# jiaxiZeng/Temporally-Consistent-Stereo-Matching

Measured on AMD Instinct MI355X. Metric: stereo-pairs/sec at 640x480 D=192, 32 GRU iters, higher is better.
Workload: dtype f32; 1 GPU; BASELINE configs[1]: 640x480 synthetic sequence len=10, D=192, 32 iters, one sequence per GPU; frames_per_rank=87, seqs_per_gpu=1, weights=key-seeded synthetic (tcs_mi355.weights)

## Files before the change

### include/tcs_mi355.h

```cpp
#ifndef TCS_MI355_H
#define TCS_MI355_H

#include <stddef.h>
#include <stdint.h>

#ifdef __cplusplus
extern "C" {
#endif

#define TCS_OK 0
#define TCS_EINVAL (-1)
#define TCS_ELAUNCH (-2)
#define TCS_EUNSUPPORTED (-3)

typedef void* tcs_stream_t;

int tcs_abi_version(void);
const char* tcs_error_string(int code);


size_t tcs_corr_level_bytes(int B, int H, int W, int level);
size_t tcs_corr_build_workspace_bytes(int B, int H, int W);

int tcs_corr_build(const float* fmap1, const float* fmap2, int B, int C, int H, int W,
                   float* pyr0, float* pyr1, float* pyr2, float* pyr3,
                   float* nat1, float* nat2, float* nat3,
                   float* cost_volume,
                   float* sparse_disp, float* sparse_cost, float* sparse_mask,
                   void* workspace, tcs_stream_t stream);
float* tcs_corr_ws_level0(void* workspace);

int tcs_corr_lookup(const float* pyr0, const float* pyr1, const float* pyr2, const float* pyr3,
                    const float* coords, int B, int H, int W, int radius, float* out,
                    unsigned long long* stamps, tcs_stream_t stream);
int tcs_corr_lookup_blocks(int B, int H, int W);

int tcs_corr_lookup_backward(const float* pyr0, const float* pyr1, const float* pyr2, const float* pyr3,
                             const float* coords, const float* grad_out, int B, int H, int W, int radius,
                             float* grad_vol, float* grad_coords, tcs_stream_t stream);

size_t tcs_corr_build_backward_scratch_bytes(int B, int C, int H, int W);
int tcs_corr_build_backward(const float* fmap1, const float* fmap2, const void* workspace, const float* grad_vol,
                            int B, int C, int H, int W, float* grad_fmap1, float* grad_fmap2, void* scratch,
                            tcs_stream_t stream);

size_t tcs_warp_workspace_bytes(int B, int C, int H, int W);

int tcs_warp_forward(const float* prev_disp, const float* prev_fmap, const float* T_rel, const float* K,
                     const float* K_inv, const float* baseline, int B, int C, int H, int W,
                     float* out_disp, float* out_fmap, float* out_mask,
                     const float* cur_fmap, float* out_cost,
// ... 301 lines not shown
```

### temporally-consistent-stereo-matching_amd/csrc/tcs_s16_ops.hip

```cpp
#include "tcs_s16.h"

__global__ __launch_bounds__(256) void k_avgpool3s2_s16(const _Float16* __restrict__ x, int G, int H, int W, int Ho, int Wo,
                                                         _Float16* __restrict__ out, int Go) {
    const int bg = blockIdx.y, b = bg / G, g = bg - b * G;
    const int p = blockIdx.x * 256 + threadIdx.x;
    if (p >= Ho * Wo) return;
    const int yo = p / Wo, xo = p - yo * Wo;
    const int Hp = H + 2, Wp = W + 2;
    const size_t plane = (size_t)Hp * Wp * 8;
    const _Float16* s = x + (((size_t)b * G + g) * 2) * plane;
    float acc[8] = {0.f, 0.f, 0.f, 0.f, 0.f, 0.f, 0.f, 0.f};
#pragma unroll
    for (int v = 0; v < 3; ++v) {
#pragma unroll
        for (int u = 0; u < 3; ++u) {
            float t[8];
            s16_load8(s + ((size_t)(2 * yo + v) * Wp + (2 * xo + u)) * 8, plane, t);
#pragma unroll
            for (int j = 0; j < 8; ++j) acc[j] += t[j];
        }
    }
#pragma unroll
    for (int j = 0; j < 8; ++j) acc[j] = acc[j] / 9.f;
    s16_store8(out + s16_unit(b, Go, g, 0, Ho + 2, Wo + 2, yo, xo), (size_t)(Ho + 2) * (Wo + 2) * 8, acc);
}

__global__ __launch_bounds__(256) void k_resize_bilinear_s16(const _Float16* __restrict__ x, int G, int H, int W, int Ho, int Wo,
                                                              _Float16* __restrict__ out, int Go) {
    const int bg = blockIdx.y, b = bg / G, g = bg - b * G;
    const int p = blockIdx.x * 256 + threadIdx.x;
    if (p >= Ho * Wo) return;
    const int yo = p / Wo, xo = p - yo * Wo;
    const float sy = Ho > 1 ? (float)(H - 1) / (float)(Ho - 1) : 0.f;
    const float sx = Wo > 1 ? (float)(W - 1) / (float)(Wo - 1) : 0.f;
    const float fy = sy * (float)yo, fx = sx * (float)xo;
    const int y0 = (int)fy, x0 = (int)fx;
    const int y1 = y0 + (y0 < H - 1), x1 = x0 + (x0 < W - 1);
    const float ly = fy - (float)y0, lx = fx - (float)x0;
    const int Hp = H + 2, Wp = W + 2;
    const size_t plane = (size_t)Hp * Wp * 8;
    const _Float16* s = x + (((size_t)b * G + g) * 2) * plane;
    float a00[8], a01[8], a10[8], a11[8], r[8];
    s16_load8(s + ((size_t)(y0 + 1) * Wp + x0 + 1) * 8, plane, a00);
    s16_load8(s + ((size_t)(y0 + 1) * Wp + x1 + 1) * 8, plane, a01);
    s16_load8(s + ((size_t)(y1 + 1) * Wp + x0 + 1) * 8, plane, a10);
    s16_load8(s + ((size_t)(y1 + 1) * Wp + x1 + 1) * 8, plane, a11);
#pragma unroll
    for (int j = 0; j < 8; ++j) r[j] = (1.f - ly) * ((1.f - lx) * a00[j] + lx * a01[j]) + ly * ((1.f - lx) * a10[j] + lx * a11[j]);
    s16_store8(out + s16_unit(b, Go, g, 0, Ho + 2, Wo + 2, yo, xo), (size_t)(Ho + 2) * (Wo + 2) * 8, r);
}

#define INS_T 256
#define INS_UPT 10

__device__ __forceinline__ void block_sum8(float* v, float* red ) {
#pragma unroll
    for (int j = 0; j < 8; ++j) v[j] = wave_sum(v[j]);
    __syncthreads();
    if ((threadIdx.x & 63) == 0) {
#pragma unroll
        for (int j = 0; j < 8; ++j) red[(threadIdx.x >> 6) * 8 + j] = v[j];
    }
    __syncthreads();
#pragma unroll
    for (int j = 0; j < 8; ++j) {
        float s = 0.f;
#pragma unroll
        for (int w = 0; w < INS_T / 64; ++w) s += red[w * 8 + j];
        v[j] = s;
    }
}

__global__ __launch_bounds__(INS_T) void k_in_stats_s16(const _Float16* __restrict__ x, int G, int H, int W, int slice_px,
                                                         float* __restrict__ partial ) {
    __shared__ float red[(INS_T / 64) * 8];
    const int bg = blockIdx.y, sl = blockIdx.x, nsl = gridDim.x;
    const int HW = H * W, Wp = W + 2;
    const size_t plane = (size_t)(H + 2) * Wp * 8;
    const _Float16* s = x + ((size_t)bg * 2) * plane;
    const int p_lo = sl * slice_px, p_hi = min(HW, p_lo + slice_px), n = p_hi - p_lo;
    float v[INS_UPT][8], sum[8] = {0.f, 0.f, 0.f, 0.f, 0.f, 0.f, 0.f, 0.f};
#pragma unroll
    for (int k = 0; k < INS_UPT; ++k) {
        const int p = p_lo + threadIdx.x + INS_T * k;
        const bool ok = p < p_hi;
        const int pc = ok ? p : p_lo;
        const int y = pc / W, xx = pc - y * W;
        s16_load8(s + ((size_t)(y + 1) * Wp + xx + 1) * 8, plane, v[k]);
#pragma unroll
        for (int j = 0; j < 8; ++j) { v[k][j] = ok ? v[k][j] : 0.f; sum[j] += v[k][j]; }
    }
    block_sum8(sum, red);
    float mean[8], m2[8] = {0.f, 0.f, 0.f, 0.f, 0.f, 0.f, 0.f, 0.f};
#pragma unroll
    for (int j = 0; j < 8; ++j) mean[j] = sum[j] / (float)n;
#pragma unroll
    for (int k = 0; k < INS_UPT; ++k) {
        const bool ok = p_lo + threadIdx.x + INS_T * k < p_hi;
#pragma unroll
        for (int j = 0; j < 8; ++j) { const float d = ok ? v[k][j] - mean[j] : 0.f; m2[j] = fmaf(d, d, m2[j]); }
    }
    block_sum8(m2, red);
    if (threadIdx.x < 8) {
        float* o = partial + ((size_t)bg * nsl + sl) * 16;
        o[threadIdx.x] = mean[threadIdx.x];
        o[8 + threadIdx.x] = m2[threadIdx.x];
    }
}

__device__ __forceinline__ float s16_act(float v, int act) {
    switch (act) {
        case TCS_ACT_RELU: return fmaxf(v, 0.f);
        case TCS_ACT_RELU_ADD_RELU: return fmaxf(v, 0.f);
        case TCS_ACT_LEAKY: return v > 0.f ? v : 0.01f * v;
        default: return v;
    }
}

__global__ __launch_bounds__(INS_T) void k_in_apply_s16(const _Float16* __restrict__ x, int G, int H, int W, int slice_px, int nsl,
                                                         const float* __restrict__ partial, float eps, int act,
                                                         const _Float16* __restrict__ addend, int Ga, _Float16* __restrict__ out, int Go) {
    const int bg = blockIdx.y, b = bg / G, g = bg - b * G;
    const int HW = H * W, Wp = W + 2;
    const size_t plane = (size_t)(H + 2) * Wp * 8;
    const int p = blockIdx.x * INS_T + threadIdx.x;
    const bool ok = p < HW;
    const int pc = ok ? p : HW - 1;
    const int y = pc / W, xx = pc - y * W;
    const size_t u = ((size_t)(y + 1) * Wp + xx + 1) * 8;
    float v[8], t[8];
    s16_load8(x + ((size_t)bg * 2) * plane + u, plane, v);
    if (addend) s16_load8(addend + (((size_t)b * Ga + g) * 2) * plane + u, plane, t);
    float n = 0.f, mean[8], m2[8];
#pragma unroll
    for (int j = 0; j < 8; ++j) { mean[j] = 0.f; m2[j] = 0.f; }
#pragma unroll 4
    for (int i = 0; i < nsl; ++i) {
        const float4* pi = reinterpret_cast<const float4*>(partial + ((size_t)bg * nsl + i) * 16);
        const float4 a0 = pi[0], a1 = pi[1], q0 = pi[2], q1 = pi[3];
        const float pm[8] = {a0.x, a0.y, a0.z, a0.w, a1.x, a1.y, a1.z, a1.w}, p2[8] = {q0.x, q0.y, q0.z, q0.w, q1.x, q1.y, q1.z, q1.w};
        const float ni = (float)(min(HW, (i + 1) * slice_px) - i * slice_px), tot = n + ni, f = ni / tot;
#pragma unroll
        for (int j = 0; j < 8; ++j) {
            const float d = pm[j] - mean[j];
            mean[j] += d * f;
            m2[j] += p2[j] + d * d * n * f;
        }
        n = tot;
    }
    if (!ok) return;
#pragma unroll
    for (int j = 0; j < 8; ++j) {
        const float rstd = 1.0f / sqrtf(m2[j] / (float)HW + eps);
        v[j] = s16_act((v[j] - mean[j]) * rstd, act) + (addend ? t[j] : 0.f);
        if (act == TCS_ACT_RELU_ADD_RELU) v[j] = fmaxf(v[j], 0.f);
    }
    s16_store8(out + (((size_t)b * Go + g) * 2) * plane + u, plane, v);
}

__global__ __launch_bounds__(INS_T) void k_in_apply_sums_s16(const _Float16* __restrict__ x, int Gt, int G, int H, int W, int C,
                                                              const long long* __restrict__ sums, float eps, int act,
                                                              const _Float16* __restrict__ addend, int Ga, _Float16* __restrict__ out, int Go) {
    const int b = blockIdx.y / G, g = blockIdx.y - b * G, bg = b * Gt + g;
    const int HW = H * W, Wp = W + 2;
    const size_t plane = (size_t)(H + 2) * Wp * 8;
    const int p = blockIdx.x * INS_T + threadIdx.x;
    if (p >= HW) return;
    const int y = p / W, xx = p - y * W;
    const size_t u = ((size_t)(y + 1) * Wp + xx + 1) * 8;
    float v[8], t[8];
    s16_load8(x + ((size_t)bg * 2) * plane + u, plane, v);
    if (addend) s16_load8(addend + (((size_t)b * Ga + g) * 2) * plane + u, plane, t);
    const long long* sp = sums + ((size_t)b * C + min(g * 8, C - 8)) * S16_IN_STRIDE;
    const double inv_n = 1.0 / (double)HW;
#pragma unroll
    for (int j = 0; j < 8; ++j) {
        const double mu = (double)sp[S16_IN_STRIDE * j] * (inv_n / 1048576.0), ex2 = (double)sp[S16_IN_STRIDE * j + 1] * (inv_n / 65536.0);
        const float mean = (float)mu, rstd = 1.0f / sqrtf(fmaxf((float)(ex2 - mu * mu), 0.f) + eps);
        const bool real = g * 8 + j < C;
        v[j] = real ? s16_act((v[j] - mean) * rstd, act) + (addend ? t[j] : 0.f) : 0.f;
        if (act == TCS_ACT_RELU_ADD_RELU) v[j] = fmaxf(v[j], 0.f);
    }
    s16_store8(out + (((size_t)b * Go + g) * 2) * plane + u, plane, v);
}

__global__ __launch_bounds__(256) void k_propagate_s16(const float* __restrict__ grad, const float* __restrict__ disp, int H, int W,
                                                        float* __restrict__ cand9, _Float16* __restrict__ out16, int Go) {
    const int b = blockIdx.y, HW = H * W;
    const int p = blockIdx.x * 256 + threadIdx.x;
    if (p >= HW) return;
// ... 114 lines not shown
}

__global__ __launch_bounds__(256) void k_s16_set_channel(const float* __restrict__ x, int H, int W, _Float16* __restrict__ out, int Go, int ch) {
    const int b = blockIdx.y, HW = H * W;
    const int p = blockIdx.x * 256 + threadIdx.x;
    if (p >= HW) return;
    const int y = p / W, xx = p - y * W;
    half2_t hi, lo;
    s16_split2(x[(size_t)b * HW + p], 0.f, hi, lo);
    _Float16* o = out + s16_unit(b, Go, ch >> 3, 0, H + 2, W + 2, y, xx) + (ch & 7);
    o[0] = hi[0];
    o[(size_t)(H + 2) * (W + 2) * 8] = lo[0];
}

extern "C" {

int tcs_avgpool3s2_s16(const void* x, int B, int groups, int H, int W, void* out, int out_groups, tcs_stream_t stream) {
    if (!x || !out || B <= 0 || groups <= 0 || out_groups < groups || H <= 0 || W <= 0) return TCS_EINVAL;
    if ((long long)B * groups > 65535) return TCS_EUNSUPPORTED;
    const int Ho = (H - 1) / 2 + 1, Wo = (W - 1) / 2 + 1;
    hipLaunchKernelGGL(k_avgpool3s2_s16, dim3(tcs_cdiv((long long)Ho * Wo, 256), B * groups), dim3(256), 0, tcs_stream(stream),
                       reinterpret_cast<const _Float16*>(x), groups, H, W, Ho, Wo, reinterpret_cast<_Float16*>(out), out_groups);
    return tcs_launch_status();
}

int tcs_resize_bilinear_s16(const void* x, int B, int groups, int H, int W, int Ho, int Wo, void* out, int out_groups, tcs_stream_t stream) {
    if (!x || !out || B <= 0 || groups <= 0 || out_groups < groups || H <= 0 || W <= 0 || Ho <= 0 || Wo <= 0) return TCS_EINVAL;
    if ((long long)B * groups > 65535) return TCS_EUNSUPPORTED;
    hipLaunchKernelGGL(k_resize_bilinear_s16, dim3(tcs_cdiv((long long)Ho * Wo, 256), B * groups), dim3(256), 0, tcs_stream(stream),
                       reinterpret_cast<const _Float16*>(x), groups, H, W, Ho, Wo, reinterpret_cast<_Float16*>(out), out_groups);
    return tcs_launch_status();
}

size_t tcs_instance_norm_s16_workspace_bytes(int B, int groups, int H, int W) {
    if (B <= 0 || groups <= 0 || H <= 0 || W <= 0) return 0;
    const int nsl = tcs_cdiv((long long)H * W, INS_T * INS_UPT);
    return (size_t)B * groups * nsl * 16 * sizeof(float);
}

int tcs_instance_norm_s16(const void* x, int B, int groups, int H, int W, float eps, int act, const void* addend, int addend_groups,
                          void* out, int out_groups, void* workspace, tcs_stream_t stream) {
    if (!x || !out || !workspace || B <= 0 || groups <= 0 || out_groups < groups || H <= 0 || W <= 0 || eps < 0.f) return TCS_EINVAL;
    if (addend && addend_groups < groups) return TCS_EINVAL;
    if (act != TCS_ACT_NONE && act != TCS_ACT_RELU && act != TCS_ACT_LEAKY && act != TCS_ACT_RELU_ADD_RELU) return TCS_EUNSUPPORTED;
    if (act == TCS_ACT_RELU_ADD_RELU && !addend) return TCS_EINVAL;
    if ((long long)B * groups > 65535) return TCS_EUNSUPPORTED;
    if (out_groups != groups || (addend && addend_groups != groups)) return TCS_EUNSUPPORTED;
    const int HW = H * W, nsl = tcs_cdiv(HW, INS_T * INS_UPT), slice = tcs_cdiv(HW, nsl);

    hipStream_t s = tcs_stream(stream);
    hipLaunchKernelGGL(k_in_stats_s16, dim3(nsl, B * groups), dim3(INS_T), 0, s, reinterpret_cast<const _Float16*>(x), groups, H, W, slice,
                       reinterpret_cast<float*>(workspace));
    hipLaunchKernelGGL(k_in_apply_s16, dim3(tcs_cdiv(HW, INS_T), B * groups), dim3(INS_T), 0, s, reinterpret_cast<const _Float16*>(x), groups, H, W,
                       slice, nsl, reinterpret_cast<const float*>(workspace), eps, act, reinterpret_cast<const _Float16*>(addend), addend_groups,
                       reinterpret_cast<_Float16*>(out), out_groups);
    return tcs_launch_status();
}

int tcs_instance_norm_apply_s16(const void* x, int B, int groups, int H, int W, int act, const void* addend, int addend_groups,
                                void* out, int out_groups, const void* in_stats, int C, float eps, tcs_stream_t stream) {
    if (!x || !out || !in_stats || B <= 0 || groups <= 0 || H <= 0 || W <= 0 || C <= 0 || C % 32 != 0 || groups * 8 < C || !(eps >= 0.f)) return TCS_EINVAL;
    if ((long long)B * (C / 8) > 65535 || (long long)H * W > (1 << 20)) return TCS_EUNSUPPORTED;
    if (act != TCS_ACT_NONE && act != TCS_ACT_RELU && act != TCS_ACT_LEAKY && act != TCS_ACT_RELU_ADD_RELU) return TCS_EUNSUPPORTED;
    if (act == TCS_ACT_RELU_ADD_RELU && !addend) return TCS_EINVAL;
    if (out_groups != groups || (addend && addend_groups != groups)) return TCS_EUNSUPPORTED;
    const int G = C / 8;
    hipLaunchKernelGGL(k_in_apply_sums_s16, dim3(tcs_cdiv((long long)H * W, INS_T), B * G), dim3(INS_T), 0, tcs_stream(stream),
                       reinterpret_cast<const _Float16*>(x), groups, G, H, W, C, reinterpret_cast<const long long*>(in_stats), eps, act,
                       reinterpret_cast<const _Float16*>(addend), addend_groups, reinterpret_cast<_Float16*>(out), out_groups);
    return tcs_launch_status();
}

int tcs_propagate_disparity_s16(const float* grad, const float* disp, int B, int H, int W, float* cand9, void* out16, int out_groups,
                                tcs_stream_t stream) {
    if (!grad || !disp || !out16 || out_groups < 4 || B <= 0 || B > 65535 || H <= 0 || W <= 0) return TCS_EINVAL;
    hipLaunchKernelGGL(k_propagate_s16, dim3(tcs_cdiv((long long)H * W, 256), B), dim3(256), 0, tcs_stream(stream), grad, disp, H, W, cand9,
                       reinterpret_cast<_Float16*>(out16), out_groups);
    return tcs_launch_status();
}

int tcs_taps_propagate_s16(const float* taps, int ntile, const float* bias2, const float* g5, float post_scale, const float* disp, int B, int H,
                           int W, float* grad_out, float* cand9, void* out16, int out_groups, tcs_stream_t stream) {
    if (!taps || !g5 || !disp || !out16 || ntile <= 0 || out_groups < 4 || B <= 0 || B > 65535 || H <= 0 || W <= 0) return TCS_EINVAL;
    auto kern = ntile == 4 ? k_taps_propagate_s16<4> : (ntile == 8 ? k_taps_propagate_s16<8> : k_taps_propagate_s16<0>);
    hipLaunchKernelGGL(kern, dim3(tcs_cdiv(W, PT_T), tcs_cdiv(H, PT_TY), B), dim3(256), 0, tcs_stream(stream), taps, ntile, bias2,
                       g5, post_scale, disp, H, W, grad_out, cand9, reinterpret_cast<_Float16*>(out16), out_groups);
    return tcs_launch_status();
}
// ... 342 lines not shown
```

### temporally-consistent-stereo-matching_amd/csrc/tcs_stencil.hip

```cpp
#include "tcs_s16.h"

__global__ __launch_bounds__(256) void k_flow_step(float* __restrict__ coords1, const float* __restrict__ delta, int W, int n,
                                                   float* __restrict__ disp_q) {
    const int i = blockIdx.x * 256 + threadIdx.x;
    if (i >= n) return;
    const float c = coords1[i] + delta[i];
    coords1[i] = c;
    disp_q[i] = (float)(i % W) - c;
}

__global__ __launch_bounds__(256) void k_grad_xy(const float* __restrict__ disp, int H, int W, float scale, float* __restrict__ grad) {
    const int b = blockIdx.y, HW = H * W;
    const int p = blockIdx.x * 256 + threadIdx.x;
    if (p >= HW) return;
    const int y = p / W, x = p - y * W;
    const float* d = disp + (size_t)b * HW;
    const float c = d[p];
    const float r = d[y * W + min(x + 1, W - 1)];
    const float dn = d[min(y + 1, H - 1) * W + x];
    grad[((size_t)b * 2 + 0) * HW + p] = scale * (r - c);
    grad[((size_t)b * 2 + 1) * HW + p] = scale * (dn - c);
}

__global__ __launch_bounds__(256) void k_grad_candidates(const float* __restrict__ disp, int H, int W, float* __restrict__ out) {
// ... 516 lines not shown
                        const float gnx = in ? gx[q] : 0.f;
                        const float gny = in ? gy[q] : 0.f;
                        c[3 * v + u] = dn + gnx * (float)(1 - u) + gny * (float)(1 - v);
                    }
                }
#pragma unroll
                for (int k = 0; k < 9; ++k) r += (double)w[k] * (double)c[k];
#pragma unroll
                for (int k = 0; k < 9; ++k) dlogits[((size_t)b * 9 + k) * HW + p] = w[k] * (float)((double)c[k] - r) * gg;
            }
        }
#pragma unroll
        for (int k = 0; k < 9; ++k) st[k][e] = t[k];
    }
    if (!dgrad) return;
    __syncthreads();
    const int ly = threadIdx.x / RB_TX, lx = threadIdx.x - ly * RB_TX;
    const int y = ty0 + ly, x = tx0 + lx;
    if (y >= H || x >= W) return;
    float ax = 0.f, ay = 0.f;
#pragma unroll
    for (int v = 0; v < 3; ++v) {
#pragma unroll
        for (int u = 0; u < 3; ++u) {
            const float t = st[3 * v + u][(ly + 2 - v) * RB_SX + (lx + 2 - u)];
            ax += t * (float)(1 - u);
            ay += t * (float)(1 - v);
        }
    }
    dgrad[((size_t)b * 2 + 0) * HW + y * W + x] = ax;
    dgrad[((size_t)b * 2 + 1) * HW + y * W + x] = ay;
}

extern "C" {

size_t tcs_tap_weights_floats(int nout, int C) {
    if (nout < 1 || nout > 2 || C <= 0) return 0;
    return (size_t)((C + 31) / 32) * 2 * 128 * 4;
}

int tcs_pack_tap_weights(const float* w_oihw, int nout, int C, int scale_log2, float* packed, tcs_stream_t stream) {
    if (!w_oihw || !packed || nout < 1 || nout > 2 || C <= 0 || scale_log2 < -60 || scale_log2 > 60) return TCS_EINVAL;
    const int nk = ((C + 31) / 32) * 2, n = nk * 128;
    hipLaunchKernelGGL(k_pack_tap_weights, dim3((n + 255) / 256), dim3(256), 0, tcs_stream(stream), w_oihw, nout, C, nk, ldexpf(1.0f, scale_log2),
                       reinterpret_cast<uint4*>(packed));
    return tcs_launch_status();
}

int tcs_taps_sum(const float* taps, int ntile, int nout, const float* bias, const float* addend, float scale, int B, int H, int W, float* out,
                 tcs_stream_t stream) {
    if (!taps || !out || ntile <= 0 || nout < 1 || nout > 2 || B <= 0 || B > 65535 || H <= 0 || W <= 0) return TCS_EINVAL;
    auto kern = ntile == 8 ? k_taps_sum<8> : (ntile == 4 ? k_taps_sum<4> : k_taps_sum<0>);
    hipLaunchKernelGGL(kern, dim3(tcs_cdiv((long long)H * W, 256), B), dim3(256), 0, tcs_stream(stream), taps, ntile, nout, bias, addend,
                       scale, H, W, out);
    return tcs_launch_status();
}

int tcs_flow_taps_step_grads(const float* coords1, const float* taps, int ntile, const float* bias, int B, int H, int W, float scale,
                             float* disp_q, float* grad, float* cands, float* delta_out, tcs_stream_t stream) {
    if (!coords1 || !taps || !disp_q || !grad || !cands || ntile <= 0 || B <= 0 || B > 65535 || H <= 0 || W <= 0) return TCS_EINVAL;
    auto kern = ntile == 8 ? k_flow_taps_step_grads<8> : (ntile == 4 ? k_flow_taps_step_grads<4> : k_flow_taps_step_grads<0>);
    hipLaunchKernelGGL(kern, dim3(tcs_cdiv(W, FT_T), tcs_cdiv(H, FT_TY), B), dim3(256), 0, tcs_stream(stream), coords1, taps,
                       ntile, bias, H, W, scale, disp_q, grad, cands, delta_out);
    return tcs_launch_status();
}

// ... 115 lines not shown
    float* ws_a = grad_flow_a ? workspace : nullptr;
    float* ws_b = grad_flow_b ? workspace + (grad_flow_a ? plane : 0) : nullptr;
    hipLaunchKernelGGL(k_upsample_flow_bwd, dim3(tcs_cdiv((long long)H * W, 64), B), dim3(256), 0, tcs_stream(stream), flow_b, mask,
                       grad_flow_a ? grad_up_a : nullptr, (grad_mask || grad_flow_b) ? grad_up_b : nullptr, H, W, grad_mask, ws_a, ws_b);
    if (grad_flow_a || grad_flow_b)
        hipLaunchKernelGGL(k_upsample_flow_bwd_gather, dim3(tcs_cdiv((long long)H * W, 256), B, 2), dim3(256), 0, tcs_stream(stream),
                           ws_a, ws_b, H, W, grad_flow_a, grad_flow_b);
    return tcs_launch_status();
}

int tcs_convex_upsample_backward(const float* flow, const float* mask, const float* grad_up, int B, int H, int W, float* grad_mask,
                                 float* grad_flow, float* workspace, tcs_stream_t stream) {
    return tcs_convex_upsample_pair_backward(flow, mask, nullptr, grad_up, B, H, W, grad_mask, nullptr, grad_flow, workspace, stream);
}

int tcs_refine_blend(const float* logits9, const float* disp_grads, const float* disp, int B, int H, int W, float* refined,
                     tcs_stream_t stream) {
    if (!logits9 || !disp_grads || !disp || !refined || B <= 0 || B > 65535 || H <= 0 || W <= 0) return TCS_EINVAL;
    hipLaunchKernelGGL(k_refine_blend, dim3(tcs_cdiv((long long)H * W, 256), B), dim3(256), 0, tcs_stream(stream), logits9, disp_grads,
                       disp, H, W, refined);
    return tcs_launch_status();
}

int tcs_refine_blend_backward(const float* logits9, const float* disp_grads, const float* disp, const float* grad_refined, int B, int H,
                              int W, float* grad_logits, float* grad_disp_grads, tcs_stream_t stream) {
    if (!logits9 || !grad_refined || B <= 0 || B > 65535 || H <= 0 || W <= 0 || (!grad_logits && !grad_disp_grads)) return TCS_EINVAL;
    if (grad_logits && (!disp_grads || !disp)) return TCS_EINVAL;
    if (tcs_cdiv(H, RB_TY) > 65535) return TCS_EUNSUPPORTED;
    hipLaunchKernelGGL(k_refine_blend_bwd, dim3(tcs_cdiv(W, RB_TX), tcs_cdiv(H, RB_TY), B), dim3(256), 0, tcs_stream(stream), logits9,
                       disp_grads, disp, grad_refined, H, W, grad_logits, grad_disp_grads);
    return tcs_launch_status();
}

int tcs_abi_version(void) { return 17; }

const char* tcs_error_string(int code) {
    switch (code) {
        case TCS_OK: return "ok";
        case TCS_EINVAL: return "invalid argument";
        case TCS_ELAUNCH: return "HIP launch failed";
        case TCS_EUNSUPPORTED: return "unsupported shape";
        default: return "unknown error";
    }
}

}

int tcs_s16_flag_take_stencil(unsigned int* out) {
    unsigned int v = 0, zero = 0;
    if (hipMemcpyFromSymbol(&v, HIP_SYMBOL(TCS_S16_FLAG_VAR), sizeof(v)) != hipSuccess) return TCS_ELAUNCH;
    if (v && hipMemcpyToSymbol(HIP_SYMBOL(TCS_S16_FLAG_VAR), &zero, sizeof(zero)) != hipSuccess) return TCS_ELAUNCH;
    *out |= v;
    return TCS_OK;
}
```

### temporally-consistent-stereo-matching_amd/tcs_mi355/graph.py

```python
from __future__ import annotations

import gc
import warnings
from typing import Callable, Dict, List, Optional

import torch

_CAPTURING = 0


_OUTPUTS_KEYS = ("up", "q", "grad", "flow_mono", "flow_init", "cost_volume")


def _flatten(temporal):
    if temporal is None:
        return []
    K, T, Tp, base, last_disp, nets, fmap1 = temporal[:7]
    return [K, T, Tp, base, last_disp, *nets, fmap1, *temporal[7:]]


def _unflatten(flat):
    if not flat:
        return None
    if flat[-1].dtype == torch.uint8:
        return _unflatten(flat[:-1]) + (flat[-1],)
    return (flat[0], flat[1], flat[2], flat[3], flat[4], list(flat[5:-1]), flat[-1])


def _wants_argmax(temporal):
    return temporal is None or len(temporal) == 8


class _no_gc:

    def __enter__(self):
        global _CAPTURING
        self.was = gc.isenabled()
        gc.disable()
        _CAPTURING += 1
# ... 94 lines not shown
            side = torch.cuda.Stream()
            side.wait_stream(torch.cuda.current_stream())
            with torch.cuda.stream(side):
                for _ in range(self.warmup):
                    run()
            torch.cuda.current_stream().wait_stream(side)
            torch.cuda.synchronize()
            entries = []
            for _ in range(2):
                g = torch.cuda.CUDAGraph()
                with _no_gc(), torch.cuda.graph(g):
                    feats = run()
                g.replay()
                entries.append(_Entry(g, static_in, feats))
            torch.cuda.synchronize()
            return entries
        except Exception as e:
            if self.strict:
                raise
            warnings.warn(f"HIP graph capture of the extract stage failed ({type(e).__name__}: {e}); running this shape with eager launches")
            torch.cuda.synchronize()
            return None

    def _launch_extract(self, si: int, image1, image2, first: bool, use_graph: bool, outputs: bool = False):
        slot = self.slots[si]
        key = self._ex_key(image1, first, outputs)
        entries = None
        if use_graph:
            if key not in self.ex:
                self.ex[key] = self._capture_extract(key, image1, image2, first, outputs)
            entries = self.ex[key]
        if entries is not None:
            e = entries[si]
            e.static_in[0].copy_(image1)
            e.static_in[1].copy_(image2)
            e.graph.replay()
            slot.feats = e.static_out
        else:
            slot.feats = self.extract_fn(image1, image2, first, outputs)
        slot.token, slot.ex_key, slot.fresh, slot.by_prefetch, slot.age = self._token(image1, image2, first, use_graph, outputs), key, True, False, 0
        self.turn = si ^ 1

    def prefetch(self, image1, image2, first: bool = False, use_graph: bool = True) -> int:
        self._check_epoch()
        token = self._token(image1, image2, first, use_graph)
        for k in (0, 1):
            if self.slots[k].fresh and self._same(self.slots[k].token, token):
                return k
        si = self._pick_slot()
        self._launch_extract(si, image1, image2, first, use_graph)
        self.slots[si].by_prefetch = True
        return si

    def _capture_refine(self, key, image1, image2, iters, flat, first, outputs=False) -> Optional[List[_Entry]]:
        ex_key = self._ex_key(image1, first, outputs)
        try:
            for si in (0, 1):
                if self.slots[si].feats is None or self.slots[si].ex_key != ex_key or self.ex.get(ex_key) is None \
                        or self.slots[si].feats is not self.ex[ex_key][si].static_out:
                    self._launch_extract(si, image1, image2, first, True, outputs=outputs)
            if self.ex.get(ex_key) is None:
                return None
            torch.cuda.synchronize()
            static_in = [t.detach().clone() if t.dtype == torch.uint8 else t.detach().float().clone() for t in flat]
            entries = []
            for si in (0, 1):
                feats = self.ex[ex_key][si].static_out
                run = lambda: self.loop_fn(feats, self.head_fn(feats, _unflatten(static_in)), iters, outputs)
# ... 23 lines not shown
            warnings.warn(f"HIP graph capture failed ({type(e).__name__}: {e}); running this shape with eager launches")
            torch.cuda.synchronize()
            return None

    def __call__(self, image1, image2, iters, temporal, use_graph: bool = True, outputs: bool = False):
        self._check_epoch()
        flat = _flatten(temporal)
        first = _wants_argmax(temporal)
        token = self._token(image1, image2, first, use_graph, outputs)
        entries = None
        if use_graph:
            key = self._rf_key(image1, iters, flat, outputs)
            if key not in self.rf:
                self.rf[key] = self._capture_refine(key, image1, image2, iters, flat, first, outputs)
            entries = self.rf[key]
            if entries is None:
                self.fell_back += 1
        si = next((k for k in (0, 1) if self.slots[k].fresh and self._same(self.slots[k].token, token)), None)
        for k in (0, 1):
            sl = self.slots[k]
            if sl.fresh and k != si:
                sl.age += 1
                if sl.age >= 2:
                    sl.fresh, sl.token = False, None
        if si is not None:
            self.prefetched += int(self.slots[si].by_prefetch)
        else:
            si = self._pick_slot()
            self._launch_extract(si, image1, image2, first, use_graph and entries is not None, outputs=outputs)
        slot = self.slots[si]
        slot.fresh, slot.token = False, None
        if entries is not None and self.ex.get(slot.ex_key) is not None and slot.feats is self.ex[slot.ex_key][si].static_out:
            e = entries[si]
            for dst, src in zip(e.static_in, flat):
                dst.copy_(src)
            e.graph.replay()
            e.graph2.replay()
            o = e.static_out
            out = {"flow": o["flow"].clone(), "flow_q": o["flow_q"].clone(), "net_list": [t.clone() for t in o["net_list"]],
                   "fmap1": o["fmap1"].clone()}
            for k in _OUTPUTS_KEYS if outputs else ():
                out[k] = o[k].clone()
        else:
            start = self.head_fn(slot.feats, temporal)
            if outputs:
                out = self.loop_fn(slot.feats, start, iters, True)
                out = dict(out, fmap1=out["fmap1"].clone(), cost_volume=out["cost_volume"].clone())
            else:
                out = self.loop_fn(slot.feats, start, iters)
                out = dict(out, fmap1=out["fmap1"].clone())
        return out
```

### temporally-consistent-stereo-matching_amd/tcs_mi355/native.py

```python
from __future__ import annotations

import ctypes as C
import os
import threading

import torch

from . import build as _build

_LIB = None
_LOCK = threading.Lock()

c_fp = C.c_void_p
c_int = C.c_int
c_f = C.c_float
c_sz = C.c_size_t


class ConvDesc(C.Structure):
    _fields_ = [
        ("src", c_fp * 4), ("src_ch", c_int * 4), ("n_src", c_int),
        ("weight", c_fp), ("bias", c_fp),
        ("B", c_int), ("H", c_int), ("W", c_int),
        ("Cin", c_int), ("Cout", c_int), ("ksize", c_int),
# ... 8 lines not shown
    ]


class ConvS16Desc(C.Structure):
    _fields_ = [
        ("src", c_fp * 4), ("src_ch", c_int * 4), ("src_groups", c_int * 4), ("n_src", c_int),
        ("weight", c_fp), ("bias", c_fp),
        ("B", c_int), ("H", c_int), ("W", c_int),
        ("Cin", c_int), ("Cout", c_int), ("ksize", c_int), ("stride", c_int),
        ("epilogue", c_int), ("act", c_int), ("post_scale", c_f), ("weight_unscale", c_f),
        ("addend", c_fp), ("addend2", c_fp), ("addend16", c_fp), ("addend16_groups", c_int), ("h", c_fp), ("h_groups", c_int), ("z", c_fp),
        ("blend_keep_z", c_int),
        ("out16", c_fp), ("out16_groups", c_int), ("out16_group_offset", c_int),
        ("out32", c_fp), ("out_ctot", c_int), ("out_coff", c_int),
        ("tile_cfg", c_int), ("addend_ctot", c_int),
        ("blend_cand", c_fp), ("blend_cand_ctot", c_int), ("blend_disp", c_fp), ("blend_refined", c_fp), ("blend_delta", c_fp),
        ("blend_coords1", c_fp), ("blend_flow_x", c_fp), ("blend_flow16", c_fp), ("blend_flow16_groups", c_int), ("blend_flow16_channel", c_int),
        ("out16b", c_fp), ("out16b_groups", c_int), ("out16_split", c_int),
        ("in_stats", c_fp), ("in_eps", c_f),
        ("tap_weights", c_fp), ("tap_out", c_fp), ("tap_nout", c_int), ("tap_tiles", c_int), ("tap_unscale", c_f),
        ("blend_warm_pyr", c_fp * 4), ("blend_warm_radius", c_int),
        ("products", c_int),
    ]


class S16Instance(C.Structure):
    _fields_ = [(n, c_int) for n in ("ksize", "stride", "epilogue", "mt", "rows", "ksteps", "nstage", "row_split", "rows_per_wave", "taps",
                                     "products", "csplit", "blocks", "threads")] + [("lds_bytes", C.c_longlong)]


SIGNATURES = {
    "tcs_abi_version": (c_int, []),
    "tcs_error_string": (C.c_char_p, [c_int]),
    "tcs_corr_level_bytes": (c_sz, [c_int, c_int, c_int, c_int]),
    "tcs_corr_build_workspace_bytes": (c_sz, [c_int, c_int, c_int]),
    "tcs_corr_build": (c_int, [c_fp, c_fp, c_int, c_int, c_int, c_int, c_fp, c_fp, c_fp, c_fp, c_fp, c_fp, c_fp, c_fp,
                               c_fp, c_fp, c_fp, c_fp, c_fp]),
    "tcs_corr_ws_level0": (c_fp, [c_fp]),
    "tcs_corr_lookup": (c_int, [c_fp, c_fp, c_fp, c_fp, c_fp, c_int, c_int, c_int, c_int, c_fp, c_fp, c_fp]),
    "tcs_corr_lookup_blocks": (c_int, [c_int, c_int, c_int]),
    "tcs_corr_lookup_backward": (c_int, [c_fp, c_fp, c_fp, c_fp, c_fp, c_fp, c_int, c_int, c_int, c_int, c_fp, c_fp, c_fp]),
    "tcs_corr_build_backward_scratch_bytes": (c_sz, [c_int, c_int, c_int, c_int]),
    "tcs_corr_build_backward": (c_int, [c_fp, c_fp, c_fp, c_fp, c_int, c_int, c_int, c_int, c_fp, c_fp, c_fp, c_fp]),
    "tcs_pose_prepare": (c_int, [c_fp, c_fp, c_fp, c_f, c_int, c_fp, c_fp, c_fp, c_fp, c_fp]),
    "tcs_pose_prepare_mixed": (c_int, [c_fp, c_fp, c_fp, c_fp, c_f, c_int, c_fp, c_fp, c_fp, c_fp, c_fp]),
    "tcs_warp_workspace_bytes": (c_sz, [c_int, c_int, c_int, c_int]),
    "tcs_warp_forward": (c_int, [c_fp, c_fp, c_fp, c_fp, c_fp, c_fp, c_int, c_int, c_int, c_int, c_fp, c_fp, c_fp, c_fp, c_fp,
                                 c_fp, c_fp]),
    "tcs_warp_geometry": (c_int, [c_fp, c_fp, c_fp, c_fp, c_fp, c_int, c_int, c_int, c_fp, c_fp, c_fp, c_fp, c_fp, c_fp]),
    "tcs_softsplat_sum": (c_int, [c_fp, c_fp, c_int, c_int, c_int, c_int, c_fp, c_fp]),
    "tcs_warp_ordered_workspace_bytes": (c_sz, [c_int, c_int, c_int, c_int]),
    "tcs_warp_forward_ordered": (c_int, [c_fp, c_fp, c_fp, c_fp, c_fp, c_fp, c_int, c_int, c_int, c_int, c_fp, c_fp, c_fp, c_fp, c_fp,
                                         c_fp, c_fp]),
    "tcs_warp_forward_mixed": (c_int, [c_fp, c_fp, c_fp, c_fp, c_fp, c_fp, c_fp, c_fp, c_fp, c_fp, c_int, c_int, c_int, c_int, c_fp,
                                       c_fp, c_fp, c_fp, c_fp, c_fp, c_fp]),
    "tcs_warp_forward_ordered_mixed": (c_int, [c_fp, c_fp, c_fp, c_fp, c_fp, c_fp, c_fp, c_fp, c_fp, c_fp, c_int, c_int, c_int, c_int,
                                               c_fp, c_fp, c_fp, c_fp, c_fp, c_fp, c_fp]),
    "tcs_softsplat_ordered_workspace_bytes": (c_sz, [c_int, c_int, c_int]),
    "tcs_softsplat_sum_ordered": (c_int, [c_fp, c_fp, c_int, c_int, c_int, c_int, c_fp, c_fp, c_fp]),
    "tcs_backward_grid": (c_int, [c_fp, c_fp, c_fp, c_fp, c_fp, c_int, c_int, c_int, c_fp, c_fp]),
    "tcs_bilinear_sample": (c_int, [c_fp, c_fp, c_int, c_int, c_int, c_int, c_int, c_int, c_fp, c_fp]),
    "tcs_bilinear_sample_mixed": (c_int, [c_fp, c_fp, c_fp, c_int, c_int, c_int, c_int, c_int, c_int, c_fp, c_fp]),
    "tcs_grid_halve": (c_int, [c_fp, c_int, c_int, c_int, c_fp, c_fp]),
    "tcs_flow_step": (c_int, [c_fp, c_fp, c_int, c_int, c_int, c_fp, c_fp]),
    "tcs_flow_step_grads": (c_int, [c_fp, c_fp, c_int, c_int, c_int, c_f, c_fp, c_fp, c_fp, c_fp]),
    "tcs_disp_gradient_xy": (c_int, [c_fp, c_int, c_int, c_int, c_f, c_fp, c_fp]),
# ... 119 lines not shown
```

### temporally-consistent-stereo-matching_amd/tcs_mi355/ops.py

```python
from __future__ import annotations

import ctypes as C
from dataclasses import dataclass
from typing import List, Optional, Sequence

import torch

from . import grouping as _grouping
from . import native as nv

ACT = {"none": 0, "relu": 1, "sigmoid": 2, "tanh": 3, "leaky": 4, "relu_add_relu": 5}
EPI_LINEAR, EPI_GRU_ZR, EPI_GRU_Q = 0, 1, 2


def _new(like: torch.Tensor, *shape) -> torch.Tensor:
    return torch.empty(shape, dtype=torch.float32, device=like.device)


def _dims4(t: torch.Tensor, name: str):
    if t.ndim != 4:
        raise ValueError(f"{name}: expected a 4-D NCHW tensor, got shape {tuple(t.shape)}")
    return tuple(int(s) for s in t.shape)


@dataclass
class CorrPyramid:
    levels: List[torch.Tensor]
    B: int
    H: int
    W: int
    workspace: torch.Tensor
    natural: Optional[List[torch.Tensor]] = None
    cost_volume: Optional[torch.Tensor] = None
    sparse: Optional[tuple] = None


def corr_build(fmap1: torch.Tensor, fmap2: torch.Tensor, argmax: bool = False, cost_volume: bool = False,
               natural: bool = False) -> CorrPyramid:
    B, Cc, H, W = _dims4(fmap1, "fmap1")
    if tuple(fmap2.shape) != (B, Cc, H, W):
        raise ValueError(f"fmap2 shape {tuple(fmap2.shape)} != fmap1 shape {tuple(fmap1.shape)}")
    L = nv.lib()
    ws_bytes = L.tcs_corr_build_workspace_bytes(B, H, W)
    ws = torch.empty(ws_bytes // 4, dtype=torch.float32, device=fmap1.device)
    levels = [_new(fmap1, B, H, W >> i, W) for i in range(4)]
    nat = [None] * 4
    if natural:
        nat = [None] + [_new(fmap1, B, H, W, W >> i) for i in range(1, 4)]
    cost = _new(fmap1, B, W, H, W) if cost_volume else None
    sp = tuple(_new(fmap1, B, 1, H, W) for _ in range(3)) if argmax else (None, None, None)
    rc = L.tcs_corr_build(nv.ptr(fmap1, "fmap1"), nv.ptr(fmap2, "fmap2"), B, Cc, H, W,
                          *[nv.ptr(t) for t in levels], nv.ptr(nat[1]), nv.ptr(nat[2]), nv.ptr(nat[3]), nv.ptr(cost),
                          nv.ptr(sp[0]), nv.ptr(sp[1]), nv.ptr(sp[2]), nv.ptr(ws), nv.stream())
    nv.check(rc, "tcs_corr_build")
    out = CorrPyramid(levels, B, H, W, ws, cost_volume=cost, sparse=sp if argmax else None)
# ... 775 lines not shown
```

Baseline: 38.47 stereo-pairs/s.

## Fuse small instance norms into one kernel and batch graph I/O copies

Instance norm on small planes now runs as one kernel per (batch, group) that computes stats and applies the normalization. This removes the separate stats pass, the partial-buffer round trip and a launch. For larger planes, the apply kernel now merges the slice partials cooperatively and shares them through LDS, instead of every thread looping over all slices, and the slice count is sized to fill the GPU. Separately, the per-tensor copy_ and clone calls around CUDA-graph replay are replaced by a single batched multi-copy kernel, cutting many small launches. The risks are lower occupancy from one block per group and small numeric changes from the different merge order.

```diff
diff --git a/include/tcs_mi355.h b/include/tcs_mi355.h
--- a/include/tcs_mi355.h
+++ b/include/tcs_mi355.h
@@ -17,6 +17,8 @@
 
 int tcs_abi_version(void);
 const char* tcs_error_string(int code);
+
+int tcs_copy_many(const void* const* src, void* const* dst, const size_t* bytes, int n, tcs_stream_t stream);
 
 
 size_t tcs_corr_level_bytes(int B, int H, int W, int level);
diff --git a/temporally-consistent-stereo-matching_amd/csrc/tcs_s16_ops.hip b/temporally-consistent-stereo-matching_amd/csrc/tcs_s16_ops.hip
--- a/temporally-consistent-stereo-matching_amd/csrc/tcs_s16_ops.hip
+++ b/temporally-consistent-stereo-matching_amd/csrc/tcs_s16_ops.hip
@@ -52,6 +52,9 @@
 
 #define INS_T 256
 #define INS_UPT 10
+#define INS_FILL 512
+#define INS_TREE 32
+#define INF_UPT 10
 
 __device__ __forceinline__ void block_sum8(float* v, float* red ) {
 #pragma unroll
@@ -82,6 +85,11 @@
     float v[INS_UPT][8], sum[8] = {0.f, 0.f, 0.f, 0.f, 0.f, 0.f, 0.f, 0.f};
 #pragma unroll
     for (int k = 0; k < INS_UPT; ++k) {
+        if (INS_T * k >= slice_px) {
+#pragma unroll
+            for (int j = 0; j < 8; ++j) v[k][j] = 0.f;
+            continue;
+        }
         const int p = p_lo + threadIdx.x + INS_T * k;
         const bool ok = p < p_hi;
         const int pc = ok ? p : p_lo;
@@ -117,9 +125,43 @@
     }
 }
 
+__device__ __forceinline__ void chan_merge(float& n, float& mean, float& m2, float nb, float mb, float qb) {
+    const float tot = n + nb, f = tot > 0.f ? nb / tot : 0.f, d = mb - mean;
+    mean += d * f;
+    m2 += qb + d * d * n * f;
+    n = tot;
+}
+
+__device__ __forceinline__ void in_merge_slices(const float* __restrict__ part , int nsl, int slice_px, int HW, float eps,
+                                                float* st , float* wred ) {
+    const int c = threadIdx.x & 7, leaf = threadIdx.x >> 3, per = (nsl + INS_TREE - 1) / INS_TREE;
+    float n = 0.f, mean = 0.f, m2 = 0.f;
+    for (int i = leaf * per; i < min(nsl, (leaf + 1) * per); ++i)
+        chan_merge(n, mean, m2, (float)(min(HW, (i + 1) * slice_px) - i * slice_px), part[(size_t)i * 16 + c], part[(size_t)i * 16 + 8 + c]);
+#pragma unroll
+    for (int o = 8; o < 64; o <<= 1) {
+        const float nb = __shfl_down(n, o, 64), mb = __shfl_down(mean, o, 64), qb = __shfl_down(m2, o, 64);
+        chan_merge(n, mean, m2, nb, mb, qb);
+    }
+    if ((threadIdx.x & 63) < 8) {
+        float* o = wred + ((threadIdx.x >> 6) * 8 + c) * 3;
+        o[0] = n; o[1] = mean; o[2] = m2;
+    }
+    __syncthreads();
+    if (threadIdx.x < 8) {
+        n = wred[c * 3]; mean = wred[c * 3 + 1]; m2 = wred[c * 3 + 2];
+#pragma unroll
+        for (int w = 1; w < INS_T / 64; ++w) chan_merge(n, mean, m2, wred[(w * 8 + c) * 3], wred[(w * 8 + c) * 3 + 1], wred[(w * 8 + c) * 3 + 2]);
+        st[c] = mean;
+        st[8 + c] = 1.0f / sqrtf(m2 / (float)HW + eps);
+    }
+    __syncthreads();
+}
+
 __global__ __launch_bounds__(INS_T) void k_in_apply_s16(const _Float16* __restrict__ x, int G, int H, int W, int slice_px, int nsl,
                                                          const float* __restrict__ partial, float eps, int act,
                                                          const _Float16* __restrict__ addend, int Ga, _Float16* __restrict__ out, int Go) {
+    __shared__ float st[16], wred[(INS_T / 64) * 8 * 3];
     const int bg = blockIdx.y, b = bg / G, g = bg - b * G;
     const int HW = H * W, Wp = W + 2;
     const size_t plane = (size_t)(H + 2) * Wp * 8;
@@ -131,31 +173,92 @@
     float v[8], t[8];
     s16_load8(x + ((size_t)bg * 2) * plane + u, plane, v);
     if (addend) s16_load8(addend + (((size_t)b * Ga + g) * 2) * plane + u, plane, t);
-    float n = 0.f, mean[8], m2[8];
-#pragma unroll
-    for (int j = 0; j < 8; ++j) { mean[j] = 0.f; m2[j] = 0.f; }
-#pragma unroll 4
-    for (int i = 0; i < nsl; ++i) {
-        const float4* pi = reinterpret_cast<const float4*>(partial + ((size_t)bg * nsl + i) * 16);
-        const float4 a0 = pi[0], a1 = pi[1], q0 = pi[2], q1 = pi[3];
-        const float pm[8] = {a0.x, a0.y, a0.z, a0.w, a1.x, a1.y, a1.z, a1.w}, p2[8] = {q0.x, q0.y, q0.z, q0.w, q1.x, q1.y, q1.z, q1.w};
-        const float ni = (float)(min(HW, (i + 1) * slice_px) - i * slice_px), tot = n + ni, f = ni / tot;
+    in_merge_slices(partial + (size_t)bg * nsl * 16, nsl, slice_px, HW, eps, st, wred);
+    if (!ok) return;
+#pragma unroll
+    for (int j = 0; j < 8; ++j) {
+        v[j] = s16_act((v[j] - st[j]) * st[8 + j], act) + (addend ? t[j] : 0.f);
+        if (act == TCS_ACT_RELU_ADD_RELU) v[j] = fmaxf(v[j], 0.f);
+    }
+    s16_store8(out + (((size_t)b * Go + g) * 2) * plane + u, plane, v);
+}
+
+template <int NT>
+__device__ __forceinline__ void block_sum8_nt(float* v, float* red ) {
+#pragma unroll
+    for (int j = 0; j < 8; ++j) v[j] = wave_sum(v[j]);
+    __syncthreads();
+    if ((threadIdx.x & 63) == 0) {
+#pragma unroll
+        for (int j = 0; j < 8; ++j) red[(threadIdx.x >> 6) * 8 + j] = v[j];
+    }
+    __syncthreads();
+#pragma unroll
+    for (int j = 0; j < 8; ++j) {
+        float s = 0.f;
+#pragma unroll
+        for (int w = 0; w < NT / 64; ++w) s += red[w * 8 + j];
+        v[j] = s;
+    }
+}
+
+template <int NT>
+__global__ __launch_bounds__(NT) void k_in_fused_s16(const _Float16* __restrict__ x, int G, int H, int W, float eps, int act,
+                                                      const _Float16* __restrict__ addend, int Ga, _Float16* __restrict__ out, int Go) {
+    __shared__ float red[(NT / 64) * 8];
+    const int bg = blockIdx.x, b = bg / G, g = bg - b * G;
+    const int HW = H * W, Wp = W + 2;
+    const size_t plane = (size_t)(H + 2) * Wp * 8;
+    const _Float16* s = x + ((size_t)bg * 2) * plane;
+    float v[INF_UPT][8], sum[8] = {0.f, 0.f, 0.f, 0.f, 0.f, 0.f, 0.f, 0.f};
+#pragma unroll
+    for (int k = 0; k < INF_UPT; ++k) {
+        if (NT * k >= HW) {
+#pragma unroll
+            for (int j = 0; j < 8; ++j) v[k][j] = 0.f;
+            continue;
+        }
+        const int p = threadIdx.x + NT * k;
+        const bool ok = p < HW;
+        const int pc = ok ? p : 0;
+        const int y = pc / W, xx = pc - y * W;
+        s16_load8(s + ((size_t)(y + 1) * Wp + xx + 1) * 8, plane, v[k]);
+#pragma unroll
+        for (int j = 0; j < 8; ++j) { v[k][j] = ok ? v[k][j] : 0.f; sum[j] += v[k][j]; }
+    }
+    block_sum8_nt<NT>(sum, red);
+    float mean[8], m2[8] = {0.f, 0.f, 0.f, 0.f, 0.f, 0.f, 0.f, 0.f};
+#pragma unroll
+    for (int j = 0; j < 8; ++j) mean[j] = sum[j] / (float)HW;
+#pragma unroll
+    for (int k = 0; k < INF_UPT; ++k) {
+        const bool ok = threadIdx.x + NT * k < HW;
+#pragma unroll
+        for (int j = 0; j < 8; ++j) { const float d = ok ? v[k][j] - mean[j] : 0.f; m2[j] = fmaf(d, d, m2[j]); }
+    }
+    block_sum8_nt<NT>(m2, red);
+    float rstd[8];
+#pragma unroll
+    for (int j = 0; j < 8; ++j) rstd[j] = 1.0f / sqrtf(m2[j] / (float)HW + eps);
+    const _Float16* a = addend ? addend + (((size_t)b * Ga + g) * 2) * plane : nullptr;
+    _Float16* o = out + (((size_t)b * Go + g) * 2) * plane;
+#pragma unroll
+    for (int k = 0; k < INF_UPT; ++k) {
+        if (NT * k >= HW) continue;
+        const int p = threadIdx.x + NT * k;
+        if (p >= HW) continue;
+        const int y = p / W, xx = p - y * W;
+        const size_t u = ((size_t)(y + 1) * Wp + xx + 1) * 8;
+        float t[8];
+        if (a) s16_load8(a + u, plane, t);
 #pragma unroll
         for (int j = 0; j < 8; ++j) {
-            const float d = pm[j] - mean[j];
-            mean[j] += d * f;
-            m2[j] += p2[j] + d * d * n * f;
-        }
-        n = tot;
-    }
-    if (!ok) return;
-#pragma unroll
-    for (int j = 0; j < 8; ++j) {
-        const float rstd = 1.0f / sqrtf(m2[j] / (float)HW + eps);
-        v[j] = s16_act((v[j] - mean[j]) * rstd, act) + (addend ? t[j] : 0.f);
-        if (act == TCS_ACT_RELU_ADD_RELU) v[j] = fmaxf(v[j], 0.f);
-    }
-    s16_store8(out + (((size_t)b * Go + g) * 2) * plane + u, plane, v);
+            float r = s16_act((v[k][j] - mean[j]) * rstd[j], act) + (a ? t[j] : 0.f);
+            if (act == TCS_ACT_RELU_ADD_RELU) r = fmaxf(r, 0.f);
+            v[k][j] = r;
+        }
+        s16_store8(o + u, plane, v[k]);
+    }
 }
 
 __global__ __launch_bounds__(INS_T) void k_in_apply_sums_s16(const _Float16* __restrict__ x, int Gt, int G, int H, int W, int C,
@@ -336,9 +439,18 @@
     return tcs_launch_status();
 }
 
+static inline void in_slices(int B, int groups, int HW, int* nsl, int* slice) {
+    int n = tcs_cdiv(INS_FILL, (long long)B * groups);
+    n = n > tcs_cdiv(HW, INS_T) ? tcs_cdiv(HW, INS_T) : n;
+    n = n < tcs_cdiv(HW, INS_T * INS_UPT) ? tcs_cdiv(HW, INS_T * INS_UPT) : n;
+    *slice = tcs_cdiv(HW, n);
+    *nsl = tcs_cdiv(HW, *slice);
+}
+
 size_t tcs_instance_norm_s16_workspace_bytes(int B, int groups, int H, int W) {
     if (B <= 0 || groups <= 0 || H <= 0 || W <= 0) return 0;
-    const int nsl = tcs_cdiv((long long)H * W, INS_T * INS_UPT);
+    int nsl, slice;
+    in_slices(B, groups, H * W, &nsl, &slice);
     return (size_t)B * groups * nsl * 16 * sizeof(float);
 }
 
@@ -350,14 +462,24 @@
     if (act == TCS_ACT_RELU_ADD_RELU && !addend) return TCS_EINVAL;
     if ((long long)B * groups > 65535) return TCS_EUNSUPPORTED;
     if (out_groups != groups || (addend && addend_groups != groups)) return TCS_EUNSUPPORTED;
-    const int HW = H * W, nsl = tcs_cdiv(HW, INS_T * INS_UPT), slice = tcs_cdiv(HW, nsl);
-
+    const int HW = H * W;
     hipStream_t s = tcs_stream(stream);
-    hipLaunchKernelGGL(k_in_stats_s16, dim3(nsl, B * groups), dim3(INS_T), 0, s, reinterpret_cast<const _Float16*>(x), groups, H, W, slice,
-                       reinterpret_cast<float*>(workspace));
-    hipLaunchKernelGGL(k_in_apply_s16, dim3(tcs_cdiv(HW, INS_T), B * groups), dim3(INS_T), 0, s, reinterpret_cast<const _Float16*>(x), groups, H, W,
-                       slice, nsl, reinterpret_cast<const float*>(workspace), eps, act, reinterpret_cast<const _Float16*>(addend), addend_groups,
-                       reinterpret_cast<_Float16*>(out), out_groups);
+    const _Float16* xs = reinterpret_cast<const _Float16*>(x);
+    const _Float16* as = reinterpret_cast<const _Float16*>(addend);
+    _Float16* os = reinterpret_cast<_Float16*>(out);
+    if (HW <= 256 * INF_UPT) {
+        hipLaunchKernelGGL(k_in_fused_s16<256>, dim3(B * groups), dim3(256), 0, s, xs, groups, H, W, eps, act, as, addend_groups, os, out_groups);
+        return tcs_launch_status();
+    }
+    if (HW <= 512 * INF_UPT) {
+        hipLaunchKernelGGL(k_in_fused_s16<512>, dim3(B * groups), dim3(512), 0, s, xs, groups, H, W, eps, act, as, addend_groups, os, out_groups);
+        return tcs_launch_status();
+    }
+    int nsl, slice;
+    in_slices(B, groups, HW, &nsl, &slice);
+    hipLaunchKernelGGL(k_in_stats_s16, dim3(nsl, B * groups), dim3(INS_T), 0, s, xs, groups, H, W, slice, reinterpret_cast<float*>(workspace));
+    hipLaunchKernelGGL(k_in_apply_s16, dim3(tcs_cdiv(HW, INS_T), B * groups), dim3(INS_T), 0, s, xs, groups, H, W, slice, nsl,
+                       reinterpret_cast<const float*>(workspace), eps, act, as, addend_groups, os, out_groups);
     return tcs_launch_status();
 }
 
diff --git a/temporally-consistent-stereo-matching_amd/csrc/tcs_stencil.hip b/temporally-consistent-stereo-matching_amd/csrc/tcs_stencil.hip
--- a/temporally-consistent-stereo-matching_amd/csrc/tcs_stencil.hip
+++ b/temporally-consistent-stereo-matching_amd/csrc/tcs_stencil.hip
@@ -572,6 +572,38 @@
     dgrad[((size_t)b * 2 + 1) * HW + y * W + x] = ay;
 }
 
+#define CM_MAX 24
+#define CM_T 256
+#define CM_BLOCKS 64
+struct cm_table {
+    const unsigned char* src[CM_MAX];
+    unsigned char* dst[CM_MAX];
+    unsigned long long bytes[CM_MAX];
+};
+
+__global__ __launch_bounds__(CM_T) void k_copy_many(const cm_table t) {
+    const unsigned char* __restrict__ s = t.src[blockIdx.y];
+    unsigned char* __restrict__ d = t.dst[blockIdx.y];
+    const size_t n = t.bytes[blockIdx.y];
+    const size_t tid = (size_t)blockIdx.x * CM_T + threadIdx.x, nth = (size_t)gridDim.x * CM_T;
+    const uintptr_t al = reinterpret_cast<uintptr_t>(s) | reinterpret_cast<uintptr_t>(d);
+    size_t done = 0;
+    if ((al & 15) == 0) {
+        const size_t n16 = n >> 4;
+        const float4* s4 = reinterpret_cast<const float4*>(s);
+        float4* d4 = reinterpret_cast<float4*>(d);
+        for (size_t i = tid; i < n16; i += nth) d4[i] = s4[i];
+        done = n16 << 4;
+    } else if ((al & 3) == 0) {
+        const size_t n4 = n >> 2;
+        const unsigned int* s1 = reinterpret_cast<const unsigned int*>(s);
+        unsigned int* d1 = reinterpret_cast<unsigned int*>(d);
+        for (size_t i = tid; i < n4; i += nth) d1[i] = s1[i];
+        done = n4 << 2;
+    }
+    for (size_t i = done + tid; i < n; i += nth) d[i] = s[i];
+}
+
 extern "C" {
 
 size_t tcs_tap_weights_floats(int nout, int C) {
@@ -753,7 +785,28 @@
     return tcs_launch_status();
 }
 
-int tcs_abi_version(void) { return 17; }
+int tcs_copy_many(const void* const* src, void* const* dst, const size_t* bytes, int n, tcs_stream_t stream) {
+    if (n < 0 || (n > 0 && (!src || !dst || !bytes))) return TCS_EINVAL;
+    for (int i = 0; i < n; ++i)
+        if (bytes[i] && (!src[i] || !dst[i])) return TCS_EINVAL;
+    for (int i0 = 0; i0 < n; i0 += CM_MAX) {
+        cm_table t;
+        size_t most = 0;
+        const int m = n - i0 < CM_MAX ? n - i0 : CM_MAX;
+        for (int i = 0; i < m; ++i) {
+            t.src[i] = reinterpret_cast<const unsigned char*>(src[i0 + i]);
+            t.dst[i] = reinterpret_cast<unsigned char*>(dst[i0 + i]);
+            t.bytes[i] = bytes[i0 + i];
+            most = bytes[i0 + i] > most ? bytes[i0 + i] : most;
+        }
+        if (!most) continue;
+        const int blocks = (int)(most / (16 * CM_T) + 1 < CM_BLOCKS ? most / (16 * CM_T) + 1 : CM_BLOCKS);
+        hipLaunchKernelGGL(k_copy_many, dim3(blocks, m), dim3(CM_T), 0, tcs_stream(stream), t);
+    }
+    return tcs_launch_status();
+}
+
+int tcs_abi_version(void) { return 18; }
 
 const char* tcs_error_string(int code) {
     switch (code) {
diff --git a/temporally-consistent-stereo-matching_amd/tcs_mi355/graph.py b/temporally-consistent-stereo-matching_amd/tcs_mi355/graph.py
--- a/temporally-consistent-stereo-matching_amd/tcs_mi355/graph.py
+++ b/temporally-consistent-stereo-matching_amd/tcs_mi355/graph.py
@@ -5,6 +5,8 @@
 from typing import Callable, Dict, List, Optional
 
 import torch
+
+from . import ops
 
 _CAPTURING = 0
 
@@ -165,8 +167,7 @@
             entries = self.ex[key]
         if entries is not None:
             e = entries[si]
-            e.static_in[0].copy_(image1)
-            e.static_in[1].copy_(image2)
+            ops.copy_many(e.static_in, (image1, image2))
             e.graph.replay()
             slot.feats = e.static_out
         else:
@@ -256,15 +257,14 @@
         slot.fresh, slot.token = False, None
         if entries is not None and self.ex.get(slot.ex_key) is not None and slot.feats is self.ex[slot.ex_key][si].static_out:
             e = entries[si]
-            for dst, src in zip(e.static_in, flat):
-                dst.copy_(src)
+            ops.copy_many(e.static_in, flat)
             e.graph.replay()
             e.graph2.replay()
             o = e.static_out
-            out = {"flow": o["flow"].clone(), "flow_q": o["flow_q"].clone(), "net_list": [t.clone() for t in o["net_list"]],
-                   "fmap1": o["fmap1"].clone()}
-            for k in _OUTPUTS_KEYS if outputs else ():
-                out[k] = o[k].clone()
+            keys = ("flow", "flow_q", "fmap1") + (_OUTPUTS_KEYS if outputs else ())
+            nets = len(o["net_list"])
+            got = ops.clone_many([*o["net_list"], *(o[k] for k in keys)])
+            out = {"net_list": got[:nets], **dict(zip(keys, got[nets:]))}
         else:
             start = self.head_fn(slot.feats, temporal)
             if outputs:
diff --git a/temporally-consistent-stereo-matching_amd/tcs_mi355/native.py b/temporally-consistent-stereo-matching_amd/tcs_mi355/native.py
--- a/temporally-consistent-stereo-matching_amd/tcs_mi355/native.py
+++ b/temporally-consistent-stereo-matching_amd/tcs_mi355/native.py
@@ -64,6 +64,7 @@
 SIGNATURES = {
     "tcs_abi_version": (c_int, []),
     "tcs_error_string": (C.c_char_p, [c_int]),
+    "tcs_copy_many": (c_int, [C.POINTER(c_fp), C.POINTER(c_fp), C.POINTER(c_sz), c_int, c_fp]),
     "tcs_corr_level_bytes": (c_sz, [c_int, c_int, c_int, c_int]),
     "tcs_corr_build_workspace_bytes": (c_sz, [c_int, c_int, c_int]),
     "tcs_corr_build": (c_int, [c_fp, c_fp, c_int, c_int, c_int, c_int, c_fp, c_fp, c_fp, c_fp, c_fp, c_fp, c_fp, c_fp,
diff --git a/temporally-consistent-stereo-matching_amd/tcs_mi355/ops.py b/temporally-consistent-stereo-matching_amd/tcs_mi355/ops.py
--- a/temporally-consistent-stereo-matching_amd/tcs_mi355/ops.py
+++ b/temporally-consistent-stereo-matching_amd/tcs_mi355/ops.py
@@ -21,6 +21,27 @@
     if t.ndim != 4:
         raise ValueError(f"{name}: expected a 4-D NCHW tensor, got shape {tuple(t.shape)}")
     return tuple(int(s) for s in t.shape)
+
+
+def copy_many(dsts: Sequence[torch.Tensor], srcs: Sequence[torch.Tensor]) -> None:
+    src_p, dst_p, nbytes = [], [], []
+    for d, s in zip(dsts, srcs):
+        if d.is_cuda and s.device == d.device and s.dtype == d.dtype and s.shape == d.shape and s.is_contiguous() and d.is_contiguous():
+            if d.numel():
+                src_p.append(s.data_ptr())
+                dst_p.append(d.data_ptr())
+                nbytes.append(d.numel() * d.element_size())
+        else:
+            d.copy_(s)
+    n = len(nbytes)
+    if n:
+        nv.check(nv.lib().tcs_copy_many((nv.c_fp * n)(*src_p), (nv.c_fp * n)(*dst_p), (nv.c_sz * n)(*nbytes), n, nv.stream()), "tcs_copy_many")
+
+
+def clone_many(srcs: Sequence[torch.Tensor]) -> List[torch.Tensor]:
+    outs = [torch.empty_like(t, memory_format=torch.contiguous_format) for t in srcs]
+    copy_many(outs, srcs)
+    return outs
 
 
 @dataclass
```

New measurement: 38.51 stereo-pairs/s (median of 4 runs). Within noise of the previous version (+0.1%).
